# finmath/finmath-lib-cuda-extensions

Measured on AMD Instinct MI355X. Metric: Monte-Carlo path-ops/sec (fused RandomVariable stream), higher is better.
Workload: dtype f32

## Files before the change

### finmath-lib-cuda-extensions_amd/host/lmm.hpp

```cpp
#pragma once
#include <algorithm>
#include <chrono>
#include <cmath>
#include <cstdio>
#include <atomic>
#include <thread>
#include <cstdlib>
#include <functional>
#include <string>
#include <vector>

#include "random_variable.hpp"

namespace fmhost { namespace lmm {


inline const std::vector<double>& atmNormalVolatilities() {
    static const std::vector<double> v = {
        0.00151, 0.00169, 0.0021, 0.00248, 0.00291, 0.00329, 0.00365, 0.004, 0.00437, 0.00466, 0.00527, 0.00571,
        0.00604, 0.00625, 0.0016, 0.00174, 0.00217, 0.00264, 0.00314, 0.00355, 0.00398, 0.00433, 0.00469,
        0.00493, 0.00569, 0.00607, 0.00627, 0.00645, 0.00182, 0.00204, 0.00238, 0.00286, 0.00339, 0.00384,
        0.00424, 0.00456, 0.00488, 0.0052, 0.0059, 0.00623, 0.0064, 0.00654, 0.00205, 0.00235, 0.00272, 0.0032,
        0.00368, 0.00406, 0.00447, 0.00484, 0.00515, 0.00544, 0.00602, 0.00629, 0.0064, 0.00646, 0.00279,
        0.00319, 0.0036, 0.00396, 0.00436, 0.00469, 0.00503, 0.0053, 0.00557, 0.00582, 0.00616, 0.00628,
        0.00638, 0.00641, 0.00379, 0.00406, 0.00439, 0.00472, 0.00504, 0.00532, 0.0056, 0.00582, 0.00602,
        0.00617, 0.0063, 0.00636, 0.00638, 0.00639, 0.00471, 0.00489, 0.00511, 0.00539, 0.00563, 0.00583, 0.006,
        0.00618, 0.0063, 0.00644, 0.00641, 0.00638, 0.00635, 0.00634, 0.00544, 0.00557, 0.00572, 0.00591,
        0.00604, 0.00617, 0.0063, 0.00641, 0.00651, 0.00661, 0.00645, 0.00634, 0.00627, 0.00624, 0.00625,
        0.00632, 0.00638, 0.00644, 0.0065, 0.00655, 0.00661, 0.00667, 0.00672, 0.00673, 0.00634, 0.00614,
        0.00599, 0.00593, 0.00664, 0.00671, 0.00675, 0.00676, 0.00676, 0.00675, 0.00676, 0.00674, 0.00672,
        0.00669, 0.00616, 0.00586, 0.00569, 0.00558, 0.00647, 0.00651, 0.00651, 0.00651, 0.00652, 0.00649,
        0.00645, 0.0064, 0.00637, 0.00631, 0.00576, 0.00534, 0.00512, 0.00495, 0.00615, 0.0062, 0.00618,
        0.00613, 0.0061, 0.00607, 0.00602, 0.00596, 0.00591, 0.00586, 0.00536, 0.00491, 0.00469, 0.0045,
        0.00578, 0.00583, 0.00579, 0.00574, 0.00567, 0.00562, 0.00556, 0.00549, 0.00545, 0.00538, 0.00493,
        0.00453, 0.00435, 0.0042, 0.00542, 0.00547, 0.00539, 0.00532, 0.00522, 0.00516, 0.0051, 0.00504, 0.005,
        0.00495, 0.00454, 0.00418, 0.00404, 0.00394 };
    return v;
}
inline const std::vector<double>& atmExpiryYears() { static const std::vector<double> v = { 1.0 / 12, 0.25, 0.5, 1, 2, 3, 4, 5, 7, 10, 15, 20, 25, 30 }; return v; }
inline const std::vector<double>& atmTenorYears()  { static const std::vector<double> v = { 1, 2, 3, 4, 5, 6, 7, 8, 9, 10, 15, 20, 25, 30 }; return v; }

struct DiscountCurve {
    std::vector<double> t{ 0.0 }, logdf{ 0.0 };
    double df(double time) const {
        if (time <= 0.0) return 1.0;
        if (time >= t.back()) return std::exp(logdf.back());
        const size_t k = (size_t)(std::upper_bound(t.begin(), t.end(), time) - t.begin());
        const double w = (time - t[k - 1]) / (t[k] - t[k - 1]);
        return std::exp(logdf[k - 1] + w * (logdf[k] - logdf[k - 1]));
    }
    double forward(double fixing, double period) const { return (df(fixing) / df(fixing + period) - 1.0) / period; }
    static DiscountCurve bootstrap() {
        const double maturities[] = { 0.5, 1, 2, 3, 4, 5, 6, 7, 8, 9, 10, 11, 12, 15, 20, 25, 30, 35, 40, 45, 50 };
        const double rates[] = { -0.00216, -0.00208, -0.00222, -0.00216, -0.0019, -0.0014, -0.00072, 0.00011, 0.00103, 0.00196, 0.00285,
                                 0.00367, 0.0044, 0.00604, 0.00733, 0.00767, 0.00773, 0.00765, 0.00752, 0.007138, 0.007 };
        DiscountCurve c;
        for (int i = 0; i < 21; ++i) {
            const double M = maturities[i], r = rates[i];
            c.t.push_back(M); c.logdf.push_back(c.logdf.back());
            auto swapValue = [&](double ld) {
                c.logdf.back() = ld;
                double annuity = 0.0;
                if (M < 1.0) annuity = M * c.df(M);
                else for (double tp = 1.0; tp <= M + 1e-9; tp += 1.0) annuity += c.df(tp);
                return 1.0 - c.df(M) - r * annuity;
            };
            double lo = -3.0, hi = 1.0;
            for (int it = 0; it < 200; ++it) { const double mid = 0.5 * (lo + hi); if (swapValue(mid) > 0) lo = mid; else hi = mid; }
            c.logdf.back() = 0.5 * (lo + hi);
        }
        return c;
    }
};

struct Swaption {
    double exercise = 0; int numberOfPeriods = 0; double swapPeriodLength = 0.5;
    std::vector<double> swapTenor; double swaprate = 0, targetVolatility = 0, annuity = 0;
};

struct Market {
    DiscountCurve curve = DiscountCurve::bootstrap();
    double lastTime = 40.0, dt = 0.5;
    TimeDiscretization timeDiscretization{ 0.0, 80, 0.5 };
    std::vector<Swaption> swaptions;
    Market() {
        const auto& vols = atmNormalVolatilities();
        for (size_t e = 0; e < atmExpiryYears().size(); ++e)
            for (size_t k = 0; k < atmTenorYears().size(); ++k) {
                const double exercise = std::round(atmExpiryYears()[e] / 0.25) * 0.25, tenor = atmTenorYears()[k];
                if (exercise < 1.0) continue;
                if (exercise + tenor > lastTime + 1e-9) continue;
                Swaption s;
                s.exercise = exercise; s.numberOfPeriods = (int)std::lround(tenor / 0.5);
                for (int p = 0; p <= s.numberOfPeriods; ++p) s.swapTenor.push_back(exercise + p * 0.5);
                double floating = 0.0, annuity = 0.0;
                for (int p = 0; p < s.numberOfPeriods; ++p) {
                    const double d = curve.df(s.swapTenor[p + 1]);
                    floating += curve.forward(s.swapTenor[p], 0.5) * 0.5 * d; annuity += 0.5 * d;
                }
                s.swaprate = floating / annuity; s.annuity = annuity;
                s.targetVolatility = vols[e * atmTenorYears().size() + k];
                swaptions.push_back(std::move(s));
            }
    }
    int numberOfLibors() const { return timeDiscretization.getNumberOfTimeSteps(); }
};

struct VolatilityModel {
    std::vector<double> grid{ 0.0, 1.0, 2.0, 5.0, 10.0, 20.0, 30.0, 40.0 };
    std::vector<double> parameter = std::vector<double>(64, 0.50 / 100);
    int bin(double x) const { int k = 0; while (k < 7 && grid[(size_t)k] < x - 1e-12) ++k; return k; }
    int parameterIndex(double time, double maturity) const { return bin(time) * 8 + bin(maturity - time); }
    double volatility(double time, double maturity) const { return maturity <= time + 1e-12 ? 0.0 : parameter[(size_t)parameterIndex(time, maturity)]; }
    std::vector<int> activeParameters(const Market& m) const {
        std::vector<char> used(64, 0);
        const auto& td = m.timeDiscretization;
        for (int i = 0; i < td.getNumberOfTimeSteps(); ++i)
            for (int j = i + 1; j < m.numberOfLibors(); ++j) used[(size_t)parameterIndex(td.getTime(i), td.getTime(j))] = 1;
        std::vector<int> idx;
        for (int k = 0; k < 64; ++k) if (used[(size_t)k]) idx.push_back(k);
        return idx;
    }
};


struct Simulation {
    std::vector<std::vector<RV>> libor;
    std::vector<RV> numeraire;
};

struct Backend {
    const RandomVariableFactory* factory = nullptr;
    const BrownianMotion* brownianMotion = nullptr;
    std::function<void()> flush = [] {};
    std::function<void(bool)> hold = [](bool) {};
    std::function<long long()> launches = [] { return 0LL; };
    std::function<std::vector<double>(const std::vector<RV>&)> averages = [](const std::vector<RV>& v) {
        std::vector<double> a; for (const RV& x : v) a.push_back(x->getAverage()); return a; };
    std::function<std::function<std::vector<double>()>(const std::vector<RV>&)> averagesAsync;
    bool expectationsRunPending = false;
    std::function<void(const std::vector<RV>&)> valuesNotNeeded;
    int chunk = 7;
    int stepsPerLaunch = 4;
    std::function<std::vector<std::vector<RV>>(const std::vector<RV>& roots, const std::vector<RV>& leafFrom, const std::vector<std::vector<RV>>& leafTo,
                                               const std::vector<std::vector<double>>* scalars)> clone;
    std::function<std::vector<double>(const std::vector<RV>& roots)> recordedScalars;
    int jacobianBatch = 1;
    bool keepAllStates = false;
    int threads = 1;
};

inline std::vector<Simulation> simulateMany(const Market& m, const std::vector<const VolatilityModel*>& vols, const Backend& be, int lastTimeIndex,
                                            const std::vector<char>* keep = nullptr) {
    const auto& td = m.timeDiscretization;
    const int n = m.numberOfLibors();
    const double delta = m.dt;
    const size_t K = vols.size();
    std::vector<Simulation> sims(K);
    for (Simulation& sim : sims) {
        sim.libor.resize((size_t)lastTimeIndex + 1);
        sim.numeraire.resize((size_t)lastTimeIndex + 1);
        sim.libor[0].resize((size_t)n);
        for (int j = 0; j < n; ++j) sim.libor[0][(size_t)j] = be.factory->createRandomVariable(0.0, m.curve.forward(td.getTime(j), delta));
        sim.numeraire[0] = be.factory->createRandomVariable(0.0, 1.0);
    }
    std::vector<RV> factorSum(K);
    const int S = std::max(1, be.stepsPerLaunch);
    static int cloneChecks = 0;
    for (int i0 = 0; i0 < lastTimeIndex;) {
        int i1 = std::min(i0 + S, lastTimeIndex);
        static const bool endAtKept = std::getenv("FMHIP_LMM_GROUPS_END_AT_KEPT") && std::getenv("FMHIP_LMM_GROUPS_END_AT_KEPT")[0] == '1';
        if (keep && endAtKept) for (int s2 = i0 + 1; s2 < i1; ++s2) if ((*keep)[(size_t)s2]) { i1 = s2; break; }
        const bool cloning = K > 1 && S > 1 && keep && be.clone && i0 >= 2;
        const size_t Krec = cloning ? 1 : K;
        if (S > 1) be.hold(true);
        for (int i = i0; i < i1; ++i) {
            const double t = td.getTime(i), dt = td.getTimeStep(i);
            const RV dW = be.brownianMotion->getBrownianIncrement(i, 0);
            for (size_t k = 0; k < Krec; ++k) {
                auto& cur = sims[k].libor[(size_t)i];
                auto& nxt = sims[k].libor[(size_t)i + 1];
                nxt.resize((size_t)n);
                for (int j = 0; j <= i && j < n; ++j) nxt[(size_t)j] = cur[(size_t)j];
                factorSum[k] = nullptr;
            }
            for (int j0 = i + 1; j0 < n; j0 += be.chunk) {
                const int j1 = std::min(n, j0 + be.chunk);
                for (size_t k = 0; k < Krec; ++k) {
                    auto& cur = sims[k].libor[(size_t)i];
                    auto& nxt = sims[k].libor[(size_t)i + 1];
                    for (int j = j0; j < j1; ++j) {
                        const double lambda = vols[k]->volatility(t, td.getTime(j));
                        const RV& L = cur[(size_t)j];
                        const RV transform = be.factory->createRandomVariable(lambda * delta)->discount(L, delta);
                        factorSum[k] = factorSum[k] ? factorSum[k]->add(transform) : transform;
                        const RV drift = factorSum[k]->mult(lambda);
                        nxt[(size_t)j] = L->addProduct(drift, dt)->addProduct(dW, lambda);
                    }
                }
                if (S == 1 && j1 - j0 == be.chunk) be.flush();
            }
            for (size_t k = 0; k < Krec; ++k)
                sims[k].numeraire[(size_t)i + 1] = sims[k].numeraire[(size_t)i]->accrue(sims[k].libor[(size_t)i][(size_t)i], delta);
            for (size_t k = 0; k < Krec; ++k) factorSum[k] = nullptr;
        }
        if (cloning) {
            std::vector<RV> roots, leafFrom;
            for (int j = i0 + 1; j < n; ++j) roots.push_back(sims[0].libor[(size_t)i1][(size_t)j]);
            for (int i = i0; i < i1; ++i) roots.push_back(sims[0].numeraire[(size_t)i + 1]);
            for (int s2 = i0 + 1; s2 < i1; ++s2)
                if (!keep || (*keep)[(size_t)s2]) for (int j = s2; j < n; ++j) roots.push_back(sims[0].libor[(size_t)s2][(size_t)j]);
            for (int j = i0; j < n; ++j) leafFrom.push_back(sims[0].libor[(size_t)i0][(size_t)j]);
            leafFrom.push_back(sims[0].numeraire[(size_t)i0]);
            auto scalarsOf = [&](const VolatilityModel& vol) {
                std::vector<double> sc;
                for (int i = i0; i < i1; ++i) {
                    const double t = td.getTime(i), dt = td.getTimeStep(i);
                    for (int j = i + 1; j < n; ++j) {
                        const double lambda = vol.volatility(t, td.getTime(j));
                        sc.push_back(delta); sc.push_back(1.0); sc.push_back(lambda * delta); sc.push_back(lambda); sc.push_back(dt); sc.push_back(lambda);
                    }
                    sc.push_back(delta);
                }
                return sc;
            };
            if (cloneChecks < 64 && be.recordedScalars) {
                ++cloneChecks;
                if (be.recordedScalars(roots) != scalarsOf(*vols[0])) throw std::runtime_error("lmm: the scalar list of the replicated Euler steps does not match the recording");
            }
            std::vector<std::vector<RV>> leafTo(K - 1);
            std::vector<std::vector<double>> scalars(K - 1);
            for (size_t k = 1; k < K; ++k) {
                for (int j = i0; j < n; ++j) leafTo[k - 1].push_back(sims[k].libor[(size_t)i0][(size_t)j]);
                leafTo[k - 1].push_back(sims[k].numeraire[(size_t)i0]);
                scalars[k - 1] = scalarsOf(*vols[k]);
            }
            const std::vector<std::vector<RV>> copies = be.clone(roots, leafFrom, leafTo, &scalars);
            for (size_t k = 1; k < K; ++k) {
                auto& nxt = sims[k].libor[(size_t)i1];
                nxt.resize((size_t)n);
                for (int j = 0; j <= i0 && j < n; ++j) nxt[(size_t)j] = sims[k].libor[(size_t)i0][(size_t)j];
                size_t r = 0;
                for (int j = i0 + 1; j < n; ++j) nxt[(size_t)j] = copies[k - 1][r++];
                for (int i = i0; i < i1; ++i) sims[k].numeraire[(size_t)i + 1] = copies[k - 1][r++];
                for (int s2 = i0 + 1; s2 < i1; ++s2)
                    if (!keep || (*keep)[(size_t)s2]) { auto& mid = sims[k].libor[(size_t)s2]; mid.resize((size_t)n); for (int j = s2; j < n; ++j) mid[(size_t)j] = copies[k - 1][r++]; }
            }
        }
        if (keep)
            for (int i = i0; i < i1; ++i)
                if (!(*keep)[(size_t)i])
                    for (size_t k = 0; k < K; ++k) { sims[k].libor[(size_t)i].clear(); sims[k].libor[(size_t)i].shrink_to_fit(); }
        if (S > 1) be.hold(false);
        be.flush();
        i0 = i1;
    }
    return sims;
}

inline Simulation simulate(const Market& m, const VolatilityModel& vol, const Backend& be, int lastTimeIndex) {
    return std::move(simulateMany(m, { &vol }, be, lastTimeIndex)[0]);
}

inline RV swaptionValue(const Market& m, const Simulation& sim, const Swaption& s) {
    const auto& td = m.timeDiscretization;
    const int exerciseIndex = td.getTimeIndex(s.exercise);
    RV value;
    for (int p = s.numberOfPeriods - 1; p >= 0; --p) {
        const int j = td.getTimeIndex(s.swapTenor[(size_t)p]);
        const RV& libor = sim.libor[(size_t)exerciseIndex][(size_t)j];
        const RV payoff = libor->sub(s.swaprate)->mult(s.swapPeriodLength);
        value = (value ? value->add(payoff) : payoff)->discount(libor, s.swapPeriodLength);
    }
    return value->floor(0.0)->div(sim.numeraire[(size_t)exerciseIndex]);
}
inline double bachelierAtmImpliedVolatility(double optionValue, double optionMaturity, double annuity) {
    return optionValue * std::sqrt(2.0 * 3.14159265358979323846) / (annuity * std::sqrt(optionMaturity));
}

struct Valuation { std::vector<double> modelVolatility; double seconds_simulation = 0, seconds_valuation = 0; long long launches_simulation = 0, launches_valuation = 0; };

struct PendingValuations {
    std::vector<std::function<std::vector<double>()>> expectations;
    std::vector<Valuation> out;
};

inline std::vector<Valuation> evaluateManyFinish(const Market& m, PendingValuations& p) {
    for (size_t k = 0; k < p.out.size(); ++k) {
        const std::vector<double> optionValues = p.expectations[k]();
        for (size_t q = 0; q < m.swaptions.size(); ++q)
            p.out[k].modelVolatility.push_back(bachelierAtmImpliedVolatility(optionValues[q], m.swaptions[q].exercise, m.swaptions[q].annuity));
    }
    return std::move(p.out);
}

inline PendingValuations evaluateManyBegin(const Market& m, const std::vector<const VolatilityModel*>& vols, const Backend& be) {
    using clk = std::chrono::steady_clock;
    const size_t K = vols.size();
    PendingValuations pending;
    std::vector<Valuation>& out = pending.out;
    out.resize(K);
    int lastIndex = 0;
    for (const Swaption& s : m.swaptions) lastIndex = std::max(lastIndex, m.timeDiscretization.getTimeIndex(s.exercise));
    const auto t0 = clk::now();
    const long long l0 = be.launches();
    std::vector<char> keep((size_t)lastIndex + 1, 0);
    for (const Swaption& s : m.swaptions) keep[(size_t)m.timeDiscretization.getTimeIndex(s.exercise)] = 1;
    const std::vector<Simulation> sims = simulateMany(m, vols, be, lastIndex, be.keepAllStates ? nullptr : &keep);
    const auto t1 = clk::now();
    const long long l1 = be.launches();
    std::vector<std::vector<RV>> values(K);
    if (K > 1 && be.clone) {
        be.hold(true);
        values[0].reserve(m.swaptions.size());
        for (const Swaption& s : m.swaptions) values[0].push_back(swaptionValue(m, sims[0], s));
        std::vector<RV> leafFrom;
        std::vector<std::vector<RV>> leafTo(K - 1);
        for (int e = 0; e <= lastIndex; ++e) {
            if (!keep[(size_t)e]) continue;
            for (size_t k = 0; k < K; ++k) {
                std::vector<RV>& dst = k == 0 ? leafFrom : leafTo[k - 1];
                for (int j = e; j < m.numberOfLibors(); ++j) dst.push_back(sims[k].libor[(size_t)e][(size_t)j]);
                dst.push_back(sims[k].numeraire[(size_t)e]);
            }
        }
        const std::vector<std::vector<RV>> copies = be.clone(values[0], leafFrom, leafTo, nullptr);
        for (size_t k = 1; k < K; ++k) values[k] = copies[k - 1];
        be.hold(false);
        if (!(be.averagesAsync && be.expectationsRunPending)) be.flush();
    } else
    for (size_t k = 0; k < K; ++k) {
        be.hold(true);
        values[k].reserve(m.swaptions.size());
        for (const Swaption& s : m.swaptions) values[k].push_back(swaptionValue(m, sims[k], s));
        be.hold(false);
        if (!(be.averagesAsync && be.expectationsRunPending)) be.flush();
    }
    if (be.valuesNotNeeded) for (size_t k = 0; k < K; ++k) be.valuesNotNeeded(values[k]);
    for (size_t k = 0; k < K; ++k) {
        if (be.averagesAsync) pending.expectations.push_back(be.averagesAsync(values[k]));
        else { const std::vector<double> now = be.averages(values[k]); pending.expectations.push_back([now] { return now; }); }
    }
    const auto t2 = clk::now();
    for (size_t k = 0; k < K; ++k) {
        out[k].launches_simulation = (l1 - l0) / (long long)K; out[k].launches_valuation = (be.launches() - l1) / (long long)K;
        out[k].seconds_simulation = std::chrono::duration<double>(t1 - t0).count() / (double)K;
        out[k].seconds_valuation = std::chrono::duration<double>(t2 - t1).count() / (double)K;
    }
    return pending;
}

inline std::vector<Valuation> evaluateMany(const Market& m, const std::vector<const VolatilityModel*>& vols, const Backend& be) {
    PendingValuations p = evaluateManyBegin(m, vols, be);
    return evaluateManyFinish(m, p);
}

inline Valuation evaluate(const Market& m, const VolatilityModel& vol, const Backend& be) {
    return std::move(evaluateMany(m, { &vol }, be)[0]);
}


struct CalibrationResult {
    VolatilityModel model; int iterations = 0, evaluations = 0;
    double meanDeviation = 0, rmsDeviation = 0, initialRms = 0, seconds = 0, seconds_simulation = 0, seconds_valuation = 0;
    std::vector<double> modelVolatility;
};

inline bool solveSymmetric(std::vector<double> A, std::vector<double> b, int n, std::vector<double>& x) {
    for (int c = 0; c < n; ++c) {
        int piv = c;
        for (int r = c + 1; r < n; ++r) if (std::fabs(A[(size_t)r * n + c]) > std::fabs(A[(size_t)piv * n + c])) piv = r;
        if (std::fabs(A[(size_t)piv * n + c]) < 1e-300) return false;
        if (piv != c) { for (int k = 0; k < n; ++k) std::swap(A[(size_t)c * n + k], A[(size_t)piv * n + k]); std::swap(b[(size_t)c], b[(size_t)piv]); }
        for (int r = c + 1; r < n; ++r) {
            const double f = A[(size_t)r * n + c] / A[(size_t)c * n + c];
            for (int k = c; k < n; ++k) A[(size_t)r * n + k] -= f * A[(size_t)c * n + k];
            b[(size_t)r] -= f * b[(size_t)c];
        }
    }
    x.assign((size_t)n, 0.0);
    for (int r = n - 1; r >= 0; --r) { double s = b[(size_t)r]; for (int k = r + 1; k < n; ++k) s -= A[(size_t)r * n + k] * x[(size_t)k]; x[(size_t)r] = s / A[(size_t)r * n + r]; }
    return true;
}

inline CalibrationResult calibrate(const Market& m, const Backend& be, int maxIterations = 200, double accuracy = 1e-7,
                                   double lambda = 0.1, double parameterStep = 1e-4, bool verbose = false) {
    using clk = std::chrono::steady_clock;
    const auto start = clk::now();
    CalibrationResult res;
    VolatilityModel vol;
    const std::vector<int> active = vol.activeParameters(m);
    const int np = (int)active.size(), nr = (int)m.swaptions.size();
    auto residuals = [&](const VolatilityModel& v, std::vector<double>& r, std::vector<double>* modelVols) {
        const Valuation val = evaluate(m, v, be);
        res.evaluations++; res.seconds_simulation += val.seconds_simulation; res.seconds_valuation += val.seconds_valuation;
        r.resize((size_t)nr);
        for (int k = 0; k < nr; ++k) r[(size_t)k] = val.modelVolatility[(size_t)k] - m.swaptions[(size_t)k].targetVolatility;
        if (modelVols) *modelVols = val.modelVolatility;
    };
    auto sumsq = [](const std::vector<double>& r) { double s = 0; for (double x : r) s += x * x; return s; };
    std::vector<double> r, rTrial, modelVols;
    residuals(vol, r, &modelVols);
    double err = sumsq(r);
    res.initialRms = std::sqrt(err / nr);
    for (int it = 0; it < maxIterations; ++it) {
        std::vector<double> J((size_t)nr * np);
        struct InFlight { int a0 = 0, a1 = 0; std::vector<VolatilityModel> bumped; PendingValuations pending; bool valid = false; };
        auto collect = [&](InFlight& f) {
            if (!f.valid) return;
            const std::vector<Valuation> vals = evaluateManyFinish(m, f.pending);
            for (int a = f.a0; a < f.a1; ++a) {
                const Valuation& val = vals[(size_t)(a - f.a0)];
                res.evaluations++; res.seconds_simulation += val.seconds_simulation; res.seconds_valuation += val.seconds_valuation;
                for (int k = 0; k < nr; ++k) J[(size_t)k * np + a] = (val.modelVolatility[(size_t)k] - m.swaptions[(size_t)k].targetVolatility - r[(size_t)k]) / parameterStep;
            }
            f.valid = false;
        };
        if (be.threads > 1 && be.jacobianBatch <= 1) {
            const auto tj0 = clk::now();
            std::vector<Valuation> column((size_t)np);
            std::vector<std::string> failures((size_t)be.threads);
            std::atomic<int> next{ 0 };
            std::vector<std::thread> pool;
            for (int t = 0; t < be.threads; ++t)
                pool.emplace_back([&, t] {
                    try {
                        for (int a = next.fetch_add(1); a < np; a = next.fetch_add(1)) {
                            VolatilityModel bumped = vol;
                            bumped.parameter[(size_t)active[(size_t)a]] += parameterStep;
                            column[(size_t)a] = evaluate(m, bumped, be);
                        }
                    } catch (const std::exception& e) { failures[(size_t)t] = e.what(); }
                });
            for (std::thread& th : pool) th.join();
            if (std::getenv("FMHIP_LMM_TIMELINE")) std::fprintf(stderr, "[lmm timeline] iteration %d: %d columns on %d threads, %.3f … %.3f ms\n", it, np, be.threads, std::chrono::duration<double, std::milli>(tj0 - start).count(), std::chrono::duration<double, std::milli>(clk::now() - start).count());
            for (const std::string& f : failures) if (!f.empty()) throw std::runtime_error("a Jacobian column failed: " + f);
            for (int a = 0; a < np; ++a) {
                const Valuation& val = column[(size_t)a];
                res.evaluations++; res.seconds_simulation += val.seconds_simulation; res.seconds_valuation += val.seconds_valuation;
                for (int k = 0; k < nr; ++k) J[(size_t)k * np + a] = (val.modelVolatility[(size_t)k] - m.swaptions[(size_t)k].targetVolatility - r[(size_t)k]) / parameterStep;
            }
        } else {
        InFlight previous;
        for (int a0 = 0; a0 < np; a0 += std::max(1, be.jacobianBatch)) {
            const int a1 = std::min(np, a0 + std::max(1, be.jacobianBatch));
            InFlight current;
            current.a0 = a0; current.a1 = a1;
            current.bumped.assign((size_t)(a1 - a0), vol);
            std::vector<const VolatilityModel*> ptrs;
            for (int a = a0; a < a1; ++a) { current.bumped[(size_t)(a - a0)].parameter[(size_t)active[(size_t)a]] += parameterStep; ptrs.push_back(&current.bumped[(size_t)(a - a0)]); }
            static const bool timeline = std::getenv("FMHIP_LMM_TIMELINE") != nullptr;
            const auto tb0 = clk::now();
            try { current.pending = evaluateManyBegin(m, ptrs, be); current.valid = true; }
            catch (const std::exception& e) {
                if (ptrs.size() == 1 || std::string(e.what()).find("allocation") == std::string::npos) throw;
                if (verbose) std::fprintf(stderr, "  batch of %zu bumps does not fit (%s): evaluating them one at a time\n", ptrs.size(), e.what());
                be.flush();
                collect(previous);
                for (int a = a0; a < a1; ++a) {
                    const Valuation val = evaluate(m, current.bumped[(size_t)(a - a0)], be);
                    res.evaluations++; res.seconds_simulation += val.seconds_simulation; res.seconds_valuation += val.seconds_valuation;
                    for (int k = 0; k < nr; ++k) J[(size_t)k * np + a] = (val.modelVolatility[(size_t)k] - m.swaptions[(size_t)k].targetVolatility - r[(size_t)k]) / parameterStep;
                }
                continue;
            }
            const auto tb1 = clk::now();
            collect(previous);
            if (timeline) std::fprintf(stderr, "[lmm timeline] iteration %d batch from %d: begin %.3f … %.3f ms, previous collected at %.3f ms\n", it, a0,
                                       std::chrono::duration<double, std::milli>(tb0 - start).count(), std::chrono::duration<double, std::milli>(tb1 - start).count(),
                                       std::chrono::duration<double, std::milli>(clk::now() - start).count());
            previous = std::move(current);
        }
        collect(previous);
        }
        std::vector<double> JtJ((size_t)np * np, 0.0), Jtr((size_t)np, 0.0);
        for (int a = 0; a < np; ++a) {
            for (int b = 0; b < np; ++b) { double s = 0; for (int k = 0; k < nr; ++k) s += J[(size_t)k * np + a] * J[(size_t)k * np + b]; JtJ[(size_t)a * np + b] = s; }
            double s = 0; for (int k = 0; k < nr; ++k) s += J[(size_t)k * np + a] * r[(size_t)k]; Jtr[(size_t)a] = -s;
        }
        bool improved = false;
        for (int attempt = 0; attempt < 8 && !improved; ++attempt) {
            std::vector<double> A = JtJ, step;
            for (int a = 0; a < np; ++a) A[(size_t)a * np + a] += lambda * std::max(JtJ[(size_t)a * np + a], 1e-12);
            if (!solveSymmetric(A, Jtr, np, step)) { lambda *= 4; continue; }
            VolatilityModel v = vol;
            for (int a = 0; a < np; ++a) v.parameter[(size_t)active[(size_t)a]] += step[(size_t)a];
            std::vector<double> mv;
            const auto tt0 = clk::now();
            residuals(v, rTrial, &mv);
            static const bool timeline2 = std::getenv("FMHIP_LMM_TIMELINE") != nullptr;
            if (timeline2) std::fprintf(stderr, "[lmm timeline] iteration %d trial %d: %.3f … %.3f ms\n", it, attempt, std::chrono::duration<double, std::milli>(tt0 - start).count(),
                                        std::chrono::duration<double, std::milli>(clk::now() - start).count());
            const double e = sumsq(rTrial);
            if (e < err) { improved = true; const double rel = (err - e) / err; vol = v; r = rTrial; err = e; modelVols = mv; lambda = std::max(lambda / 3.0, 1e-9); if (rel < accuracy) it = maxIterations; }
            else lambda *= 4.0;
        }
        res.iterations++;
        if (verbose) std::fprintf(stderr, "  LM iteration %d: rms %.6e  lambda %.3g  evaluations %d\n", res.iterations, std::sqrt(err / nr), lambda, res.evaluations);
        if (!improved || std::sqrt(err / nr) < accuracy) break;
    }
    res.model = vol; res.modelVolatility = modelVols;
    double sum = 0; for (double x : r) sum += x;
    res.meanDeviation = sum / nr; res.rmsDeviation = std::sqrt(err / nr);
    res.seconds = std::chrono::duration<double>(clk::now() - start).count();
    return res;
}

}}
```

### finmath-lib-cuda-extensions_amd/host/lmm_hip_main.cpp

```cpp
#include <fstream>
#include <thread>
#include <csignal>
#include <execinfo.h>
#include <unistd.h>
#include <rccl/rccl.h>
#include "lmm_main_common.hpp"
#include "hip_backend.hpp"
using namespace fmhost;

static void ncclCheck(ncclResult_t r, const char* what) {
    if (r != ncclSuccess) throw std::runtime_error(std::string(what) + ": " + ncclGetErrorString(r));
}

static void fatalSignal(int sig) {
    void* frames[64];
    const int n = backtrace(frames, 64);
    const char msg[] = "lmm_hip: fatal signal, call stack:\n";
    (void)!write(2, msg, sizeof msg - 1);
    backtrace_symbols_fd(frames, n, 2);
    signal(sig, SIG_DFL);
    raise(sig);
}

int main(int argc, char** argv) {
    if (std::getenv("FMHIP_BACKTRACE")) { signal(SIGABRT, fatalSignal); signal(SIGSEGV, fatalSignal); signal(SIGBUS, fatalSignal); }
    const lmm::Options o = lmm::parseOptions(argc, argv);
    try {
        if (!o.devices.empty()) check(fmhip_init_devices(o.devices.data(), (int)o.devices.size()));
        else check(fmhip_init(-1));
        check(fmhip_set_fusion(1, nullptr));
        RandomVariableHipFactory factory;
        lmm::Market m;
        const int64_t pathOffset = o.pathOffset + (int64_t)o.rank * o.paths;
        BrownianMotionHip philox(m.timeDiscretization, 1, o.paths, o.seed, pathOffset);
        BrownianMotionFromMersenneRandomNumbers mersenne(m.timeDiscretization, 1, o.paths, (int)o.seed, &factory);
        if (o.brownian == "mersenne" && o.world > 1) throw std::runtime_error("--brownian mersenne is a sequential stream: not available with --world > 1 (mersenne-device is)");
        BrownianMotionFromMersenneRandomNumbersHip mersenneDevice(m.timeDiscretization, 1, o.paths, (int)o.seed, pathOffset);
        lmm::Backend be = makeHipBackend(&factory, (o.brownian == "mersenne") ? static_cast<const BrownianMotion*>(&mersenne)
                                                 : (o.brownian == "mersenne-device") ? static_cast<const BrownianMotion*>(&mersenneDevice) : &philox,
                                         o.chunk, o.stepsPerLaunch, o.jacobianBatch);

        if (o.finmathLike) {
            be.flush = [] {}; be.hold = [](bool) {}; be.clone = nullptr; be.recordedScalars = nullptr; be.averagesAsync = nullptr; be.expectationsRunPending = false;
            be.averages = [](const std::vector<RV>& v) { std::vector<double> a; for (const RV& x : v) a.push_back(x->getAverage()); return a; };
            be.jacobianBatch = 1; be.stepsPerLaunch = 1; be.chunk = 1 << 30; be.keepAllStates = true;
            if (o.threads > 1) {
                if (!o.devices.empty() || o.world > 1) throw std::runtime_error("--threads: one device, one process");
                check(fmhip_set_thread_engines(1, nullptr));
                be.threads = o.threads;
            }
        } else if (o.threads > 1) throw std::runtime_error("--threads belongs to --finmath-like (the native driver batches its Jacobian columns instead)");
        if (o.releaseLagMs > 0.0 || o.releaseLagBytes > 0) ReleaseLag::instance().start(o.releaseLagMs, (size_t)o.releaseLagBytes);
        ncclComm_t comm = nullptr;
        std::vector<std::pair<double*, hipEvent_t>> sparePinned;
        fmhip_vec sums = 0;
        long long collectives = 0;
        double collective_seconds = 0.0;
        if (o.world > 1 || !o.ncclIdFile.empty()) {
            if (o.ncclIdFile.empty()) throw std::runtime_error("--world needs --nccl-id-file");
            struct IdFile { uint64_t magic, nonce; ncclUniqueId id; } rec{};
            const uint64_t MAGIC = 0x464d4e43434c4944ull;
            if (o.rank == 0) {
                std::remove(o.ncclIdFile.c_str());
                rec.magic = MAGIC; rec.nonce = (uint64_t)o.ncclNonce;
                ncclCheck(ncclGetUniqueId(&rec.id), "ncclGetUniqueId");
                { std::ofstream f(o.ncclIdFile + ".tmp", std::ios::binary); f.write((const char*)&rec, sizeof rec); }
                std::rename((o.ncclIdFile + ".tmp").c_str(), o.ncclIdFile.c_str());
            } else {
                for (int tries = 0; ; ++tries) {
                    std::ifstream f(o.ncclIdFile, std::ios::binary);
                    if (f && f.read((char*)&rec, sizeof rec) && f.gcount() == (std::streamsize)sizeof rec && rec.magic == MAGIC && rec.nonce == (uint64_t)o.ncclNonce) break;
                    if (tries > 6000) throw std::runtime_error("timed out waiting for " + o.ncclIdFile);
                    std::this_thread::sleep_for(std::chrono::milliseconds(10));
                }
            }
            const ncclUniqueId id = rec.id;
            ncclCheck(ncclCommInitRank(&comm, o.world, id, o.rank), "ncclCommInitRank");
            if (o.rank == 0) std::remove(o.ncclIdFile.c_str());
            const int count = (int)m.swaptions.size();
            check(fmhip_vec_create_uninitialized((int64_t)count * 8 * o.world, &sums));
            void* stream = nullptr; check(fmhip_get_stream(&stream));
            const int64_t totalPaths = (int64_t)o.world * o.paths;
            const int world = o.world, rank = o.rank;
            struct Flight {
                fmhip_vec dev = 0; double* host = nullptr; hipEvent_t ev = nullptr;
                std::vector<std::pair<double*, hipEvent_t>>* spare = nullptr;
                ~Flight() { if (dev) fmhip_vec_release(dev); if (host && ev && spare) spare->push_back({ host, ev }); }
            };
            std::vector<std::pair<double*, hipEvent_t>>* const spare = &sparePinned;
            { const char* e = std::getenv("FMHIP_LMM_SHARDED_FROM_LAUNCHES"); be.expectationsRunPending = !(e && e[0] == '0'); }
            be.averagesAsync = [=, &collectives, &collective_seconds](const std::vector<RV>& v) -> std::function<std::vector<double>()> {
                std::vector<fmhip_vec> h;
                for (const RV& x : v) {
                    auto p = dynamic_cast<const RandomVariableHip*>(x.get());
                    if (!p || p->isDeterministic()) throw std::runtime_error("sharded expectation of a non-device value");
                    h.push_back(p->deviceVector().handle());
                }
                if ((int)h.size() != count) throw std::runtime_error("sharded expectation: unexpected product count");
                auto f = std::make_shared<Flight>();
                const size_t doubles = (size_t)count * 4 * (size_t)world;
                check(fmhip_vec_create_uninitialized((int64_t)doubles * 2, &f->dev));
                f->spare = spare;
                if (!spare->empty()) { f->host = spare->back().first; f->ev = spare->back().second; spare->pop_back(); }
                else if (hipHostMalloc((void**)&f->host, doubles * 8, hipHostMallocDefault) != hipSuccess || hipEventCreateWithFlags(&f->ev, hipEventDisableTiming) != hipSuccess)
                    throw std::runtime_error("pinned memory / event for a sharded expectation");
                void* dev = nullptr; check(fmhip_vec_device_ptr(f->dev, &dev));
                double* all = (double*)dev;
                check(fmhip_reduce_moments_batch_device(h.data(), count, nullptr, all + (size_t)rank * count * 4));
                ncclCheck(ncclAllGather(all + (size_t)rank * count * 4, all, (size_t)count * 4, ncclDouble, comm, (hipStream_t)stream), "ncclAllGather");
                if (hipMemcpyAsync(f->host, all, doubles * 8, hipMemcpyDeviceToHost, (hipStream_t)stream) != hipSuccess || hipEventRecord(f->ev, (hipStream_t)stream) != hipSuccess)
                    throw std::runtime_error("enqueueing the read-back of a sharded expectation");
                ++collectives;
                return [f, count, world, totalPaths, &collective_seconds] {
                    const auto t0 = std::chrono::steady_clock::now();
                    if (hipEventSynchronize(f->ev) != hipSuccess) throw std::runtime_error("waiting for a sharded expectation");
                    collective_seconds += std::chrono::duration<double>(std::chrono::steady_clock::now() - t0).count();
                    std::vector<double> out((size_t)count);
                    for (int k = 0; k < count; ++k) {
                        double total = 0.0;
                        for (int r = 0; r < world; ++r) total += f->host[((size_t)r * count + k) * 4];
                        out[(size_t)k] = total / (double)totalPaths;
                    }
                    return out;
                };
            };
            be.averages = [=, &collectives, &collective_seconds](const std::vector<RV>& v) {
                std::vector<fmhip_vec> h;
                for (const RV& x : v) {
                    auto p = dynamic_cast<const RandomVariableHip*>(x.get());
                    if (!p || p->isDeterministic()) throw std::runtime_error("sharded expectation of a non-device value");
                    h.push_back(p->deviceVector().handle());
                }
                if ((int)h.size() != count) throw std::runtime_error("sharded expectation: unexpected product count");
                void* dev = nullptr; check(fmhip_vec_device_ptr(sums, &dev));
                double* all = (double*)dev;
                check(fmhip_reduce_moments_batch_device(h.data(), count, nullptr, all + (size_t)rank * count * 4));
                const auto t0 = std::chrono::steady_clock::now();
                ncclCheck(ncclAllGather(all + (size_t)rank * count * 4, all, (size_t)count * 4, ncclDouble, comm, (hipStream_t)stream), "ncclAllGather");
                ++collectives;
                std::vector<float> raw((size_t)count * 8 * world);
                check(fmhip_vec_read_float(sums, raw.data(), (int64_t)raw.size()));
                collective_seconds += std::chrono::duration<double>(std::chrono::steady_clock::now() - t0).count();
                std::vector<double> out((size_t)count);
                for (int k = 0; k < count; ++k) {
                    double total = 0.0;
                    for (int r = 0; r < world; ++r) { double s; std::memcpy(&s, &raw[((size_t)r * count + k) * 8], 8); total += s; }
                    out[(size_t)k] = total / (double)totalPaths;
                }
                return out;
            };
        }

        if (o.mode == "evaluate" && o.warmupEvaluations > 0) {
            lmm::VolatilityModel vol;
            (void)lmm::evaluateMany(m, std::vector<const lmm::VolatilityModel*>((size_t)o.warmupEvaluations, &vol), be);
            check(fmhip_jit_wait());
        }
        fmhip_pool_stats_t s0; check(fmhip_pool_stats(&s0));
        int64_t bytes0 = 0; check(fmhip_traffic_stats(&bytes0, nullptr));
        if (o.profile) check(fmhip_profile_enable(1));
        auto extra = [&] {
            fmhip_pool_stats_t s; check(fmhip_pool_stats(&s));
            char name[128] = { 0 }; int cus = 0; int64_t hbm = 0; fmhip_device_info(name, 128, &cus, &hbm);
            int64_t jc = 0, jf = 0, jp = 0, jd = 0; double js = 0.0; fmhip_jit_stats(&jc, &jf, &jp, &js, &jd);
            int64_t bytes1 = 0, jl = 0; fmhip_traffic_stats(&bytes1, &jl);
            std::string prof;
            if (o.profile) {
                double ms = 0.0; int64_t nl = 0; fmhip_profile_read(&ms, &nl);
                char pb[256];
                std::snprintf(pb, sizeof pb, ", \"profiled_launches\": %lld, \"kernel_ms_total\": %.3f, \"achieved_GBps\": %.1f",
                              (long long)nl, ms, ms > 0 ? (double)(bytes1 - bytes0) / (ms * 1e-3) / 1e9 : 0.0);
                prof = pb;
            }
            char buf[768];
            std::snprintf(buf, sizeof buf, ", \"kernel_launches\": %lld, \"path_ops\": %.6e, \"device_bytes_reserved\": %lld, \"device\": \"%s\", "
                          "\"world\": %d, \"rank\": %d, \"total_paths\": %lld, \"rccl_collectives\": %lld, \"rccl_collective_seconds\": %.6f, "
                          "\"specialised_kernels\": %lld, \"specialisations_from_disk_cache\": %lld, \"specialisations_pending\": %lld, \"specialisation_seconds\": %.3f, "
                          "\"algorithmic_bytes\": %lld, \"specialised_launches\": %lld",
                          (long long)(s.n_kernel_launches - s0.n_kernel_launches), (double)(s.n_ops_executed - s0.n_ops_executed) * (double)o.paths,
                          (long long)s.bytes_reserved, name, o.world, o.rank, (long long)o.world * (long long)o.paths, collectives, collective_seconds,
                          (long long)jc, (long long)jd, (long long)jp, js, (long long)(bytes1 - bytes0), (long long)jl);
            std::string lag;
            if (ReleaseLag::instance().on()) {
                const ReleaseLag::Stats ls = ReleaseLag::instance().stats();
                char lb[384];
                std::snprintf(lb, sizeof lb, ", \"release_lag\": {\"collect_every_ms\": %.3f, \"collect_at_bytes\": %lld, \"handles_queued\": %lld, \"handles_released\": %lld, "
                              "\"collections\": %lld, \"collections_forced_by_out_of_memory\": %lld, \"peak_dead_handles\": %lld}",
                              o.releaseLagMs, o.releaseLagBytes, ls.queued, ls.released, ls.collections, ls.forcedCollections, ls.peakQueue);
                lag = lb;
            }
            fmhip_engine_stats_t es; check(fmhip_engine_stats(&es));
            char eb[768];
            std::snprintf(eb, sizeof eb, ", \"engine\": {\"interpreter_launches\": %lld, \"algorithmic_bytes_written\": %lld, \"values_deferred\": %lld, \"values_deferred_now\": %lld, "
                          "\"values_demanded\": %lld, \"peak_bytes_reserved\": %lld, \"late_releases_while_waiting\": %lld, \"late_releases_at_once\": %lld, \"late_release_seconds\": %.3f, "
                          "\"merged_launches\": %lld, \"merged_chains\": %lld, \"common_rows\": %lld, \"rolled_launches\": %lld}",
                          (long long)es.interpreter_launches, (long long)es.algorithmic_bytes_written, (long long)es.values_deferred, (long long)es.values_deferred_now,
                          (long long)es.values_demanded, (long long)es.peak_bytes_reserved, (long long)es.late_releases_while_waiting, (long long)es.late_releases_at_once, (double)es.late_release_nanoseconds * 1e-9,
                          (long long)es.merged_launches, (long long)es.merged_chains, (long long)es.common_rows, (long long)es.rolled_launches);
            return std::string(buf) + prof + lag + eb;
        };
        if (o.rank == 0) lmm::runAndReport(o, be, "hip", extra);
        else { lmm::Options quiet = o; quiet.verbose = false; lmm::runAndReport(quiet, be, "hip", extra); }
        if (sums) fmhip_vec_release(sums);
        ReleaseLag::instance().stop();
        be = lmm::Backend();
        for (auto& pe : sparePinned) { (void)hipHostFree(pe.first); (void)hipEventDestroy(pe.second); }
        if (comm) ncclCommDestroy(comm);
        check(fmhip_shutdown());
    } catch (const std::exception& e) { std::fprintf(stderr, "lmm_hip[rank %d]: %s\n", o.rank, e.what()); return 1; }
    return 0;
}
```

### finmath-lib-cuda-extensions_amd/host/lmm_main_common.hpp

```cpp
#pragma once
#include <vector>
#include <cstdlib>
#include <cstring>
#include <string>
#include "lmm.hpp"

namespace fmhost { namespace lmm {

struct Options {
    int64_t paths = 10000; int64_t seed = 31415; int maxIterations = 200; std::string mode = "calibrate"; bool verbose = false;
    int64_t pathOffset = 0; int evaluations = 1;
    int warmupEvaluations = 0;
    int world = 1, rank = 0; std::string ncclIdFile; long long ncclNonce = 0;
    std::vector<int> devices;
    int chunk = 0;
    int stepsPerLaunch = 0;
    int jacobianBatch = 0;
    std::string brownian = "philox";
    int threads = 1;
    double releaseLagMs = 0.0;
    long long releaseLagBytes = 0;
    bool finmathLike = false;
    bool profile = false;
};
inline Options parseOptions(int argc, char** argv) {
    Options o;
    for (int i = 1; i < argc; ++i) {
        const std::string a = argv[i];
        auto next = [&]() -> const char* { if (i + 1 >= argc) { std::fprintf(stderr, "missing value for %s\n", a.c_str()); std::exit(2); } return argv[++i]; };
        if (a == "--paths") o.paths = std::atoll(next());
        else if (a == "--seed") o.seed = std::atoll(next());
        else if (a == "--max-iterations") o.maxIterations = std::atoi(next());
        else if (a == "--mode") o.mode = next();
        else if (a == "--evaluations") o.evaluations = std::atoi(next());
        else if (a == "--warmup-evaluations") o.warmupEvaluations = std::atoi(next());
        else if (a == "--path-offset") o.pathOffset = std::atoll(next());
        else if (a == "--world") o.world = std::atoi(next());
        else if (a == "--devices") { std::string list = next(); size_t p0 = 0; while (p0 <= list.size()) { const size_t q = list.find(',', p0); o.devices.push_back(std::atoi(list.substr(p0, q == std::string::npos ? std::string::npos : q - p0).c_str())); if (q == std::string::npos) break; p0 = q + 1; } }
        else if (a == "--rank") o.rank = std::atoi(next());
        else if (a == "--nccl-id-file") o.ncclIdFile = next();
        else if (a == "--nccl-nonce") o.ncclNonce = std::atoll(next());
        else if (a == "--profile") o.profile = true;
        else if (a == "--finmath-like") o.finmathLike = true;
        else if (a == "--threads") o.threads = std::atoi(next());
        else if (a == "--release-lag") o.releaseLagMs = std::atof(next());
        else if (a == "--release-lag-bytes") o.releaseLagBytes = std::atoll(next());
        else if (a == "--brownian") o.brownian = next();
        else if (a == "--jacobian-batch") o.jacobianBatch = std::atoi(next());
        else if (a == "--chunk") o.chunk = std::atoi(next());
        else if (a == "--steps-per-launch") o.stepsPerLaunch = std::atoi(next());
        else if (a == "--verbose") o.verbose = true;
        else { std::fprintf(stderr, "unknown option %s\n", a.c_str()); std::exit(2); }
    }
    return o;
}

inline void runAndReport(const Options& o, const Backend& be, const char* backendName, const std::function<std::string()>& extraJson) {
    Market m;
    if (o.mode == "evaluate") {
        VolatilityModel vol;
        Valuation v;
        double sim = 0, val = 0;
        const int K = std::max(1, o.jacobianBatch);
        for (int k = 0; k < o.evaluations; k += K) {
            const int kk = std::min(K, o.evaluations - k);
            const std::vector<Valuation> vs = evaluateMany(m, std::vector<const VolatilityModel*>((size_t)kk, &vol), be);
            for (const Valuation& x : vs) { sim += x.seconds_simulation; val += x.seconds_valuation; }
            v = vs.back();
        }
        std::printf("{\"backend\": \"%s\", \"mode\": \"evaluate\", \"paths\": %lld, \"swaptions\": %zu, \"evaluations\": %d, "
                    "\"seconds_simulation_per_evaluation\": %.6f, \"seconds_valuation_per_evaluation\": %.6f, \"launches_simulation\": %lld, \"launches_valuation\": %lld%s, \"model_volatility\": [",
                    backendName, (long long)o.paths, m.swaptions.size(), o.evaluations, sim / o.evaluations, val / o.evaluations, v.launches_simulation, v.launches_valuation, extraJson().c_str());
        for (size_t k = 0; k < v.modelVolatility.size(); ++k) std::printf("%s%.17g", k ? ", " : "", v.modelVolatility[k]);
        std::printf("]}\n");
        return;
    }
    const CalibrationResult r = calibrate(m, be, o.maxIterations, 1e-7, 0.1, 1e-4, o.verbose);
    std::printf("{\"backend\": \"%s\", \"mode\": \"calibrate\", \"paths\": %lld, \"swaptions\": %zu, \"active_parameters\": %zu, "
                "\"iterations\": %d, \"evaluations\": %d, \"seconds\": %.4f, \"seconds_simulation\": %.4f, \"seconds_valuation\": %.4f, "
                "\"initial_rms\": %.6e, \"rms_deviation\": %.6e, \"mean_deviation\": %.6e%s, \"parameters\": [",
                backendName, (long long)o.paths, m.swaptions.size(), VolatilityModel().activeParameters(m).size(), r.iterations, r.evaluations,
                r.seconds, r.seconds_simulation, r.seconds_valuation, r.initialRms, r.rmsDeviation, r.meanDeviation, extraJson().c_str());
    for (size_t k = 0; k < r.model.parameter.size(); ++k) std::printf("%s%.17g", k ? ", " : "", r.model.parameter[k]);
    std::printf("]}\n");
}

}}
```

Before: 4220 billion.

## Restart Jacobian column simulations from base point at the first divergent Euler step

During calibration, each perturbed volatility model is compared against the base model to find the first time step where volatilities differ. Euler groups before that step reuse the base point's retained LIBOR and numeraire states. Columns that never diverge reuse the base option values, and only the swaptions affected are revalued. This is meant to skip redundant path simulation and valuation work in finite-difference Jacobians, at the cost of retaining group-start states in memory and handling variable product counts in the sharded reductions.

```diff
diff --git a/finmath-lib-cuda-extensions_amd/host/lmm.hpp b/finmath-lib-cuda-extensions_amd/host/lmm.hpp
--- a/finmath-lib-cuda-extensions_amd/host/lmm.hpp
+++ b/finmath-lib-cuda-extensions_amd/host/lmm.hpp
@@ -6,7 +6,10 @@
 #include <atomic>
 #include <thread>
 #include <cstdlib>
+#include <cstring>
 #include <functional>
+#include <limits>
+#include <memory>
 #include <string>
 #include <vector>
 
@@ -147,19 +150,74 @@
     std::function<std::vector<double>(const std::vector<RV>& roots)> recordedScalars;
     int jacobianBatch = 1;
     bool keepAllStates = false;
+    bool restartFromBase = true;
+    bool everySetReduces = false;
     int threads = 1;
 };
 
+
+constexpr int NEVER = std::numeric_limits<int>::max();
+
+inline int divergenceStep(const Market& m, const VolatilityModel& a, const VolatilityModel& b, int lastTimeIndex) {
+    const auto& td = m.timeDiscretization;
+    for (int d = 0; d < lastTimeIndex; ++d)
+        for (int j = d + 1; j < m.numberOfLibors(); ++j) {
+            const double x = a.volatility(td.getTime(d), td.getTime(j)), y = b.volatility(td.getTime(d), td.getTime(j));
+            if (std::memcmp(&x, &y, sizeof x) != 0) return d;
+        }
+    return NEVER;
+}
+
+inline bool groupsEndAtKept() {
+    static const bool on = std::getenv("FMHIP_LMM_GROUPS_END_AT_KEPT") && std::getenv("FMHIP_LMM_GROUPS_END_AT_KEPT")[0] == '1';
+    return on;
+}
+inline std::vector<int> eulerGroupStarts(const Backend& be, int lastTimeIndex, const std::vector<char>* keep) {
+    const int S = std::max(1, be.stepsPerLaunch);
+    std::vector<int> starts;
+    for (int i0 = 0; i0 < lastTimeIndex;) {
+        int i1 = std::min(i0 + S, lastTimeIndex);
+        if (keep && groupsEndAtKept()) for (int s2 = i0 + 1; s2 < i1; ++s2) if ((*keep)[(size_t)s2]) { i1 = s2; break; }
+        starts.push_back(i0);
+        i0 = i1;
+    }
+    starts.push_back(lastTimeIndex);
+    return starts;
+}
+
+struct BasePoint {
+    VolatilityModel model;
+    int lastTimeIndex = -1;
+    std::vector<int> groupStarts;
+    Simulation states;
+    std::vector<double> optionValues;
+    bool valid() const { return lastTimeIndex >= 0 && !optionValues.empty(); }
+};
+
 inline std::vector<Simulation> simulateMany(const Market& m, const std::vector<const VolatilityModel*>& vols, const Backend& be, int lastTimeIndex,
-                                            const std::vector<char>* keep = nullptr) {
+                                            const std::vector<char>* keep = nullptr, const BasePoint* base = nullptr, const std::vector<int>* diverges = nullptr,
+                                            bool retainGroupStarts = false, long long* groupsFromBase = nullptr) {
     const auto& td = m.timeDiscretization;
     const int n = m.numberOfLibors();
     const double delta = m.dt;
     const size_t K = vols.size();
+    const std::vector<int> starts = eulerGroupStarts(be, lastTimeIndex, keep);
+    std::vector<int> joinAt(K, 0);
+    if (base && diverges && base->lastTimeIndex == lastTimeIndex && base->groupStarts == starts)
+        for (size_t k = 0; k < K; ++k) {
+            const int d = (*diverges)[k];
+            if (d == NEVER) { joinAt[k] = NEVER; continue; }
+            size_t g = 0;
+            while (g + 2 < starts.size() && starts[g + 1] <= d) ++g;
+            joinAt[k] = starts[g];
+            if (groupsFromBase) *groupsFromBase += (long long)g;
+        }
     std::vector<Simulation> sims(K);
-    for (Simulation& sim : sims) {
+    for (size_t k = 0; k < K; ++k) {
+        Simulation& sim = sims[k];
         sim.libor.resize((size_t)lastTimeIndex + 1);
         sim.numeraire.resize((size_t)lastTimeIndex + 1);
+        if (joinAt[k] != 0) continue;
         sim.libor[0].resize((size_t)n);
         for (int j = 0; j < n; ++j) sim.libor[0][(size_t)j] = be.factory->createRandomVariable(0.0, m.curve.forward(td.getTime(j), delta));
         sim.numeraire[0] = be.factory->createRandomVariable(0.0, 1.0);
@@ -167,17 +225,25 @@
     std::vector<RV> factorSum(K);
     const int S = std::max(1, be.stepsPerLaunch);
     static int cloneChecks = 0;
-    for (int i0 = 0; i0 < lastTimeIndex;) {
-        int i1 = std::min(i0 + S, lastTimeIndex);
-        static const bool endAtKept = std::getenv("FMHIP_LMM_GROUPS_END_AT_KEPT") && std::getenv("FMHIP_LMM_GROUPS_END_AT_KEPT")[0] == '1';
-        if (keep && endAtKept) for (int s2 = i0 + 1; s2 < i1; ++s2) if ((*keep)[(size_t)s2]) { i1 = s2; break; }
-        const bool cloning = K > 1 && S > 1 && keep && be.clone && i0 >= 2;
-        const size_t Krec = cloning ? 1 : K;
+    for (size_t g = 0; g + 1 < starts.size(); ++g) {
+        const int i0 = starts[g], i1 = starts[g + 1];
+        std::vector<size_t> active;
+        for (size_t k = 0; k < K; ++k) {
+            if (joinAt[k] == i0 && i0 > 0) {
+                if (base->states.libor[(size_t)i0].size() != (size_t)n || !base->states.numeraire[(size_t)i0]) throw std::runtime_error("lmm: the base point has no state at a group start");
+                sims[k].libor[(size_t)i0] = base->states.libor[(size_t)i0];
+                sims[k].numeraire[(size_t)i0] = base->states.numeraire[(size_t)i0];
+            }
+            if (joinAt[k] <= i0) active.push_back(k);
+        }
+        if (active.empty()) continue;
+        const bool cloning = active.size() > 1 && S > 1 && keep && be.clone && i0 >= 2;
+        const std::vector<size_t> recorded = cloning ? std::vector<size_t>{ active[0] } : active;
         if (S > 1) be.hold(true);
         for (int i = i0; i < i1; ++i) {
             const double t = td.getTime(i), dt = td.getTimeStep(i);
             const RV dW = be.brownianMotion->getBrownianIncrement(i, 0);
-            for (size_t k = 0; k < Krec; ++k) {
+            for (size_t k : recorded) {
                 auto& cur = sims[k].libor[(size_t)i];
                 auto& nxt = sims[k].libor[(size_t)i + 1];
                 nxt.resize((size_t)n);
@@ -186,7 +252,7 @@
             }
             for (int j0 = i + 1; j0 < n; j0 += be.chunk) {
                 const int j1 = std::min(n, j0 + be.chunk);
-                for (size_t k = 0; k < Krec; ++k) {
+                for (size_t k : recorded) {
                     auto& cur = sims[k].libor[(size_t)i];
                     auto& nxt = sims[k].libor[(size_t)i + 1];
                     for (int j = j0; j < j1; ++j) {
@@ -200,18 +266,19 @@
                 }
                 if (S == 1 && j1 - j0 == be.chunk) be.flush();
             }
-            for (size_t k = 0; k < Krec; ++k)
+            for (size_t k : recorded)
                 sims[k].numeraire[(size_t)i + 1] = sims[k].numeraire[(size_t)i]->accrue(sims[k].libor[(size_t)i][(size_t)i], delta);
-            for (size_t k = 0; k < Krec; ++k) factorSum[k] = nullptr;
+            for (size_t k : recorded) factorSum[k] = nullptr;
         }
         if (cloning) {
+            const Simulation& first = sims[active[0]];
             std::vector<RV> roots, leafFrom;
-            for (int j = i0 + 1; j < n; ++j) roots.push_back(sims[0].libor[(size_t)i1][(size_t)j]);
-            for (int i = i0; i < i1; ++i) roots.push_back(sims[0].numeraire[(size_t)i + 1]);
+            for (int j = i0 + 1; j < n; ++j) roots.push_back(first.libor[(size_t)i1][(size_t)j]);
+            for (int i = i0; i < i1; ++i) roots.push_back(first.numeraire[(size_t)i + 1]);
             for (int s2 = i0 + 1; s2 < i1; ++s2)
-                if (!keep || (*keep)[(size_t)s2]) for (int j = s2; j < n; ++j) roots.push_back(sims[0].libor[(size_t)s2][(size_t)j]);
-            for (int j = i0; j < n; ++j) leafFrom.push_back(sims[0].libor[(size_t)i0][(size_t)j]);
-            leafFrom.push_back(sims[0].numeraire[(size_t)i0]);
+                if (!keep || (*keep)[(size_t)s2]) for (int j = s2; j < n; ++j) roots.push_back(first.libor[(size_t)s2][(size_t)j]);
+            for (int j = i0; j < n; ++j) leafFrom.push_back(first.libor[(size_t)i0][(size_t)j]);
+            leafFrom.push_back(first.numeraire[(size_t)i0]);
             auto scalarsOf = [&](const VolatilityModel& vol) {
                 std::vector<double> sc;
                 for (int i = i0; i < i1; ++i) {
@@ -226,34 +293,36 @@
             };
             if (cloneChecks < 64 && be.recordedScalars) {
                 ++cloneChecks;
-                if (be.recordedScalars(roots) != scalarsOf(*vols[0])) throw std::runtime_error("lmm: the scalar list of the replicated Euler steps does not match the recording");
-            }
-            std::vector<std::vector<RV>> leafTo(K - 1);
-            std::vector<std::vector<double>> scalars(K - 1);
-            for (size_t k = 1; k < K; ++k) {
-                for (int j = i0; j < n; ++j) leafTo[k - 1].push_back(sims[k].libor[(size_t)i0][(size_t)j]);
-                leafTo[k - 1].push_back(sims[k].numeraire[(size_t)i0]);
-                scalars[k - 1] = scalarsOf(*vols[k]);
+                if (be.recordedScalars(roots) != scalarsOf(*vols[active[0]])) throw std::runtime_error("lmm: the scalar list of the replicated Euler steps does not match the recording");
+            }
+            const size_t C = active.size() - 1;
+            std::vector<std::vector<RV>> leafTo(C);
+            std::vector<std::vector<double>> scalars(C);
+            for (size_t c = 0; c < C; ++c) {
+                const size_t k = active[c + 1];
+                for (int j = i0; j < n; ++j) leafTo[c].push_back(sims[k].libor[(size_t)i0][(size_t)j]);
+                leafTo[c].push_back(sims[k].numeraire[(size_t)i0]);
+                scalars[c] = scalarsOf(*vols[k]);
             }
             const std::vector<std::vector<RV>> copies = be.clone(roots, leafFrom, leafTo, &scalars);
-            for (size_t k = 1; k < K; ++k) {
+            for (size_t c = 0; c < C; ++c) {
+                const size_t k = active[c + 1];
                 auto& nxt = sims[k].libor[(size_t)i1];
                 nxt.resize((size_t)n);
                 for (int j = 0; j <= i0 && j < n; ++j) nxt[(size_t)j] = sims[k].libor[(size_t)i0][(size_t)j];
                 size_t r = 0;
-                for (int j = i0 + 1; j < n; ++j) nxt[(size_t)j] = copies[k - 1][r++];
-                for (int i = i0; i < i1; ++i) sims[k].numeraire[(size_t)i + 1] = copies[k - 1][r++];
+                for (int j = i0 + 1; j < n; ++j) nxt[(size_t)j] = copies[c][r++];
+                for (int i = i0; i < i1; ++i) sims[k].numeraire[(size_t)i + 1] = copies[c][r++];
                 for (int s2 = i0 + 1; s2 < i1; ++s2)
-                    if (!keep || (*keep)[(size_t)s2]) { auto& mid = sims[k].libor[(size_t)s2]; mid.resize((size_t)n); for (int j = s2; j < n; ++j) mid[(size_t)j] = copies[k - 1][r++]; }
+                    if (!keep || (*keep)[(size_t)s2]) { auto& mid = sims[k].libor[(size_t)s2]; mid.resize((size_t)n); for (int j = s2; j < n; ++j) mid[(size_t)j] = copies[c][r++]; }
             }
         }
         if (keep)
             for (int i = i0; i < i1; ++i)
-                if (!(*keep)[(size_t)i])
+                if (!(*keep)[(size_t)i] && !(retainGroupStarts && i == i0))
                     for (size_t k = 0; k < K; ++k) { sims[k].libor[(size_t)i].clear(); sims[k].libor[(size_t)i].shrink_to_fit(); }
         if (S > 1) be.hold(false);
         be.flush();
-        i0 = i1;
     }
     return sims;
 }
@@ -278,68 +347,140 @@
     return optionValue * std::sqrt(2.0 * 3.14159265358979323846) / (annuity * std::sqrt(optionMaturity));
 }
 
-struct Valuation { std::vector<double> modelVolatility; double seconds_simulation = 0, seconds_valuation = 0; long long launches_simulation = 0, launches_valuation = 0; };
+struct Valuation { std::vector<double> modelVolatility, optionValues; double seconds_simulation = 0, seconds_valuation = 0; long long launches_simulation = 0, launches_valuation = 0; };
 
 struct PendingValuations {
     std::vector<std::function<std::vector<double>()>> expectations;
     std::vector<Valuation> out;
+    long long eulerGroupsFromBase = 0, expectationsFromBase = 0;
 };
 
 inline std::vector<Valuation> evaluateManyFinish(const Market& m, PendingValuations& p) {
     for (size_t k = 0; k < p.out.size(); ++k) {
-        const std::vector<double> optionValues = p.expectations[k]();
+        p.out[k].optionValues = p.expectations[k]();
         for (size_t q = 0; q < m.swaptions.size(); ++q)
-            p.out[k].modelVolatility.push_back(bachelierAtmImpliedVolatility(optionValues[q], m.swaptions[q].exercise, m.swaptions[q].annuity));
+            p.out[k].modelVolatility.push_back(bachelierAtmImpliedVolatility(p.out[k].optionValues[q], m.swaptions[q].exercise, m.swaptions[q].annuity));
     }
     return std::move(p.out);
 }
 
-inline PendingValuations evaluateManyBegin(const Market& m, const std::vector<const VolatilityModel*>& vols, const Backend& be) {
+inline int lastExerciseIndex(const Market& m) {
+    int lastIndex = 0;
+    for (const Swaption& s : m.swaptions) lastIndex = std::max(lastIndex, m.timeDiscretization.getTimeIndex(s.exercise));
+    return lastIndex;
+}
+
+inline PendingValuations evaluateManyBegin(const Market& m, const std::vector<const VolatilityModel*>& vols, const Backend& be,
+                                           const BasePoint* base = nullptr, BasePoint* retain = nullptr) {
     using clk = std::chrono::steady_clock;
-    const size_t K = vols.size();
+    const size_t K = vols.size(), Q = m.swaptions.size();
     PendingValuations pending;
     std::vector<Valuation>& out = pending.out;
     out.resize(K);
-    int lastIndex = 0;
-    for (const Swaption& s : m.swaptions) lastIndex = std::max(lastIndex, m.timeDiscretization.getTimeIndex(s.exercise));
+    const int lastIndex = lastExerciseIndex(m);
     const auto t0 = clk::now();
     const long long l0 = be.launches();
     std::vector<char> keep((size_t)lastIndex + 1, 0);
-    for (const Swaption& s : m.swaptions) keep[(size_t)m.timeDiscretization.getTimeIndex(s.exercise)] = 1;
-    const std::vector<Simulation> sims = simulateMany(m, vols, be, lastIndex, be.keepAllStates ? nullptr : &keep);
+    std::vector<int> exerciseIndex(Q);
+    for (size_t q = 0; q < Q; ++q) { exerciseIndex[q] = m.timeDiscretization.getTimeIndex(m.swaptions[q].exercise); keep[(size_t)exerciseIndex[q]] = 1; }
+    const std::vector<char>* keepList = be.keepAllStates ? nullptr : &keep;
+    if (!keepList) retain = nullptr;
+    if (base && !(keepList && base->valid() && base->lastTimeIndex == lastIndex && base->optionValues.size() == Q
+                  && base->groupStarts == eulerGroupStarts(be, lastIndex, keepList))) base = nullptr;
+    std::vector<size_t> live;
+    std::vector<int> diverges;
+    std::vector<const VolatilityModel*> liveVols;
+    for (size_t k = 0; k < K; ++k) {
+        int d = base ? divergenceStep(m, base->model, *vols[k], lastIndex) : -1;
+        if (d == NEVER && be.everySetReduces) d = lastIndex - 1;
+        if (d == NEVER) { pending.expectationsFromBase += (long long)Q; continue; }
+        live.push_back(k); diverges.push_back(d); liveVols.push_back(vols[k]);
+    }
+    const size_t KL = live.size();
+    const std::vector<Simulation> sims = KL == 0 ? std::vector<Simulation>()
+        : simulateMany(m, liveVols, be, lastIndex, keepList, base, base ? &diverges : nullptr, retain != nullptr, &pending.eulerGroupsFromBase);
     const auto t1 = clk::now();
     const long long l1 = be.launches();
-    std::vector<std::vector<RV>> values(K);
-    if (K > 1 && be.clone) {
+    auto valued = [&](size_t c, size_t q) { return diverges[c] < exerciseIndex[q]; };
+    std::vector<std::vector<RV>> values(KL, std::vector<RV>(Q));
+    if (KL > 1 && be.clone) {
         be.hold(true);
-        values[0].reserve(m.swaptions.size());
-        for (const Swaption& s : m.swaptions) values[0].push_back(swaptionValue(m, sims[0], s));
-        std::vector<RV> leafFrom;
-        std::vector<std::vector<RV>> leafTo(K - 1);
-        for (int e = 0; e <= lastIndex; ++e) {
-            if (!keep[(size_t)e]) continue;
-            for (size_t k = 0; k < K; ++k) {
-                std::vector<RV>& dst = k == 0 ? leafFrom : leafTo[k - 1];
-                for (int j = e; j < m.numberOfLibors(); ++j) dst.push_back(sims[k].libor[(size_t)e][(size_t)j]);
-                dst.push_back(sims[k].numeraire[(size_t)e]);
-            }
-        }
-        const std::vector<std::vector<RV>> copies = be.clone(values[0], leafFrom, leafTo, nullptr);
-        for (size_t k = 1; k < K; ++k) values[k] = copies[k - 1];
+        std::vector<int> dates;
+        for (int e = 0; e <= lastIndex; ++e) if (keep[(size_t)e]) dates.push_back(e);
+        auto setsAt = [&](int e) { std::vector<size_t> a; for (size_t c = 0; c < KL; ++c) if (diverges[c] < e) a.push_back(c); return a; };
+        for (size_t d0 = 0; d0 < dates.size();) {
+            const std::vector<size_t> sets = setsAt(dates[d0]);
+            size_t d1 = d0 + 1;
+            while (d1 < dates.size() && setsAt(dates[d1]) == sets) ++d1;
+            const int eFrom = dates[d0], eTo = dates[d1 - 1];
+            d0 = d1;
+            if (sets.empty()) continue;
+            std::vector<RV> roots;
+            std::vector<size_t> rootProduct;
+            for (size_t q = 0; q < Q; ++q)
+                if (exerciseIndex[q] >= eFrom && exerciseIndex[q] <= eTo) { values[sets[0]][q] = swaptionValue(m, sims[sets[0]], m.swaptions[q]); roots.push_back(values[sets[0]][q]); rootProduct.push_back(q); }
+            if (sets.size() == 1) continue;
+            std::vector<RV> leafFrom;
+            std::vector<std::vector<RV>> leafTo(sets.size() - 1);
+            for (int e = eFrom; e <= eTo; ++e) {
+                if (!keep[(size_t)e]) continue;
+                for (size_t i = 0; i < sets.size(); ++i) {
+                    std::vector<RV>& dst = i == 0 ? leafFrom : leafTo[i - 1];
+                    for (int j = e; j < m.numberOfLibors(); ++j) dst.push_back(sims[sets[i]].libor[(size_t)e][(size_t)j]);
+                    dst.push_back(sims[sets[i]].numeraire[(size_t)e]);
+                }
+            }
+            const std::vector<std::vector<RV>> copies = be.clone(roots, leafFrom, leafTo, nullptr);
+            for (size_t i = 1; i < sets.size(); ++i)
+                for (size_t r = 0; r < roots.size(); ++r) values[sets[i]][rootProduct[r]] = copies[i - 1][r];
+        }
         be.hold(false);
         if (!(be.averagesAsync && be.expectationsRunPending)) be.flush();
     } else
-    for (size_t k = 0; k < K; ++k) {
+    for (size_t c = 0; c < KL; ++c) {
         be.hold(true);
-        values[k].reserve(m.swaptions.size());
-        for (const Swaption& s : m.swaptions) values[k].push_back(swaptionValue(m, sims[k], s));
+        for (size_t q = 0; q < Q; ++q) if (valued(c, q)) values[c][q] = swaptionValue(m, sims[c], m.swaptions[q]);
         be.hold(false);
         if (!(be.averagesAsync && be.expectationsRunPending)) be.flush();
     }
-    if (be.valuesNotNeeded) for (size_t k = 0; k < K; ++k) be.valuesNotNeeded(values[k]);
-    for (size_t k = 0; k < K; ++k) {
-        if (be.averagesAsync) pending.expectations.push_back(be.averagesAsync(values[k]));
-        else { const std::vector<double> now = be.averages(values[k]); pending.expectations.push_back([now] { return now; }); }
+    std::vector<std::vector<RV>> own(KL);
+    std::vector<std::vector<size_t>> ownProduct(KL);
+    for (size_t c = 0; c < KL; ++c)
+        for (size_t q = 0; q < Q; ++q)
+            if (values[c][q]) { own[c].push_back(values[c][q]); ownProduct[c].push_back(q); }
+    values.clear();
+    if (be.valuesNotNeeded) for (size_t c = 0; c < KL; ++c) if (!own[c].empty()) be.valuesNotNeeded(own[c]);
+    const std::shared_ptr<const std::vector<double>> baseValues = base ? std::make_shared<const std::vector<double>>(base->optionValues) : nullptr;
+    pending.expectations.resize(K);
+    for (size_t k = 0; k < K; ++k) pending.expectations[k] = [baseValues] { return *baseValues; };
+    for (size_t c = 0; c < KL; ++c) {
+        pending.expectationsFromBase += (long long)(Q - own[c].size());
+        std::function<std::vector<double>()> part;
+        if (own[c].empty()) part = [] { return std::vector<double>(); };
+        else if (be.averagesAsync) part = be.averagesAsync(own[c]);
+        else { const std::vector<double> now = be.averages(own[c]); part = [now] { return now; }; }
+        const std::vector<size_t> where = ownProduct[c];
+        pending.expectations[live[c]] = [part, where, baseValues, Q] {
+            std::vector<double> all = baseValues ? *baseValues : std::vector<double>(Q, 0.0);
+            const std::vector<double> got = part();
+            for (size_t i = 0; i < where.size(); ++i) all[where[i]] = got[i];
+            return all;
+        };
+    }
+    if (retain && KL == 1 && K == 1) {
+        retain->model = *vols[0]; retain->lastTimeIndex = lastIndex; retain->groupStarts = eulerGroupStarts(be, lastIndex, keepList);
+        retain->optionValues.clear();
+        retain->states = Simulation();
+        retain->states.libor.resize((size_t)lastIndex + 1);
+        retain->states.numeraire.resize((size_t)lastIndex + 1);
+        std::vector<char> wanted = keep;
+        for (int i0 : retain->groupStarts) wanted[(size_t)i0] = 1;
+        for (int i = 0; i <= lastIndex; ++i) {
+            if (!wanted[(size_t)i]) continue;
+            retain->states.libor[(size_t)i] = sims[0].libor[(size_t)i];
+            for (int j = 0; j < i && j < (int)retain->states.libor[(size_t)i].size(); ++j) retain->states.libor[(size_t)i][(size_t)j] = nullptr;
+            retain->states.numeraire[(size_t)i] = sims[0].numeraire[(size_t)i];
+        }
     }
     const auto t2 = clk::now();
     for (size_t k = 0; k < K; ++k) {
@@ -364,6 +505,7 @@
     VolatilityModel model; int iterations = 0, evaluations = 0;
     double meanDeviation = 0, rmsDeviation = 0, initialRms = 0, seconds = 0, seconds_simulation = 0, seconds_valuation = 0;
     std::vector<double> modelVolatility;
+    long long jacobianColumnsNotSimulated = 0, eulerGroupsFromBase = 0, expectationsFromBase = 0;
 };
 
 inline bool solveSymmetric(std::vector<double> A, std::vector<double> b, int n, std::vector<double>& x) {
@@ -391,8 +533,14 @@
     VolatilityModel vol;
     const std::vector<int> active = vol.activeParameters(m);
     const int np = (int)active.size(), nr = (int)m.swaptions.size();
-    auto residuals = [&](const VolatilityModel& v, std::vector<double>& r, std::vector<double>* modelVols) {
-        const Valuation val = evaluate(m, v, be);
+    static const bool restartKnob = !(std::getenv("FMHIP_LMM_RESTART") && std::getenv("FMHIP_LMM_RESTART")[0] == '0');
+    const bool restart = restartKnob && be.restartFromBase && !be.keepAllStates && be.threads <= 1;
+    const int lastIndex = lastExerciseIndex(m);
+    BasePoint base, candidate;
+    auto residuals = [&](const VolatilityModel& v, std::vector<double>& r, std::vector<double>* modelVols, BasePoint* retain) {
+        PendingValuations p = evaluateManyBegin(m, { &v }, be, nullptr, retain);
+        const Valuation val = std::move(evaluateManyFinish(m, p)[0]);
+        if (retain) retain->optionValues = val.optionValues;
         res.evaluations++; res.seconds_simulation += val.seconds_simulation; res.seconds_valuation += val.seconds_valuation;
         r.resize((size_t)nr);
         for (int k = 0; k < nr; ++k) r[(size_t)k] = val.modelVolatility[(size_t)k] - m.swaptions[(size_t)k].targetVolatility;
@@ -400,17 +548,19 @@
     };
     auto sumsq = [](const std::vector<double>& r) { double s = 0; for (double x : r) s += x * x; return s; };
     std::vector<double> r, rTrial, modelVols;
-    residuals(vol, r, &modelVols);
+    residuals(vol, r, &modelVols, restart ? &base : nullptr);
     double err = sumsq(r);
     res.initialRms = std::sqrt(err / nr);
     for (int it = 0; it < maxIterations; ++it) {
         std::vector<double> J((size_t)nr * np);
-        struct InFlight { int a0 = 0, a1 = 0; std::vector<VolatilityModel> bumped; PendingValuations pending; bool valid = false; };
+        struct InFlight { std::vector<int> columns; std::vector<VolatilityModel> bumped; PendingValuations pending; bool valid = false; };
         auto collect = [&](InFlight& f) {
             if (!f.valid) return;
+            res.eulerGroupsFromBase += f.pending.eulerGroupsFromBase; res.expectationsFromBase += f.pending.expectationsFromBase;
             const std::vector<Valuation> vals = evaluateManyFinish(m, f.pending);
-            for (int a = f.a0; a < f.a1; ++a) {
-                const Valuation& val = vals[(size_t)(a - f.a0)];
+            for (size_t c = 0; c < f.columns.size(); ++c) {
+                const int a = f.columns[c];
+                const Valuation& val = vals[c];
                 res.evaluations++; res.seconds_simulation += val.seconds_simulation; res.seconds_valuation += val.seconds_valuation;
                 for (int k = 0; k < nr; ++k) J[(size_t)k * np + a] = (val.modelVolatility[(size_t)k] - m.swaptions[(size_t)k].targetVolatility - r[(size_t)k]) / parameterStep;
             }
@@ -441,24 +591,44 @@
                 for (int k = 0; k < nr; ++k) J[(size_t)k * np + a] = (val.modelVolatility[(size_t)k] - m.swaptions[(size_t)k].targetVolatility - r[(size_t)k]) / parameterStep;
             }
         } else {
+        const BasePoint* from = restart && base.valid() ? &base : nullptr;
+        std::vector<int> columns;
+        for (int a = 0; a < np; ++a) {
+            if (from) {
+                VolatilityModel bumped = vol;
+                bumped.parameter[(size_t)active[(size_t)a]] += parameterStep;
+                if (!be.everySetReduces && divergenceStep(m, from->model, bumped, lastIndex) == NEVER) {
+                    res.evaluations++; res.jacobianColumnsNotSimulated++; res.expectationsFromBase += nr;
+                    for (int k = 0; k < nr; ++k) {
+                        const double modelVolatility = bachelierAtmImpliedVolatility(from->optionValues[(size_t)k], m.swaptions[(size_t)k].exercise, m.swaptions[(size_t)k].annuity);
+                        J[(size_t)k * np + a] = (modelVolatility - m.swaptions[(size_t)k].targetVolatility - r[(size_t)k]) / parameterStep;
+                    }
+                    continue;
+                }
+            }
+            columns.push_back(a);
+        }
         InFlight previous;
-        for (int a0 = 0; a0 < np; a0 += std::max(1, be.jacobianBatch)) {
-            const int a1 = std::min(np, a0 + std::max(1, be.jacobianBatch));
+        const size_t batch = (size_t)std::max(1, be.jacobianBatch);
+        for (size_t c0 = 0; c0 < columns.size(); c0 += batch) {
+            const size_t c1 = std::min(columns.size(), c0 + batch);
+            const int a0 = columns[c0];
             InFlight current;
-            current.a0 = a0; current.a1 = a1;
-            current.bumped.assign((size_t)(a1 - a0), vol);
+            current.columns.assign(columns.begin() + (std::ptrdiff_t)c0, columns.begin() + (std::ptrdiff_t)c1);
+            current.bumped.assign(c1 - c0, vol);
             std::vector<const VolatilityModel*> ptrs;
-            for (int a = a0; a < a1; ++a) { current.bumped[(size_t)(a - a0)].parameter[(size_t)active[(size_t)a]] += parameterStep; ptrs.push_back(&current.bumped[(size_t)(a - a0)]); }
+            for (size_t c = c0; c < c1; ++c) { current.bumped[c - c0].parameter[(size_t)active[(size_t)columns[c]]] += parameterStep; ptrs.push_back(&current.bumped[c - c0]); }
             static const bool timeline = std::getenv("FMHIP_LMM_TIMELINE") != nullptr;
             const auto tb0 = clk::now();
-            try { current.pending = evaluateManyBegin(m, ptrs, be); current.valid = true; }
+            try { current.pending = evaluateManyBegin(m, ptrs, be, from); current.valid = true; }
             catch (const std::exception& e) {
                 if (ptrs.size() == 1 || std::string(e.what()).find("allocation") == std::string::npos) throw;
                 if (verbose) std::fprintf(stderr, "  batch of %zu bumps does not fit (%s): evaluating them one at a time\n", ptrs.size(), e.what());
                 be.flush();
                 collect(previous);
-                for (int a = a0; a < a1; ++a) {
-                    const Valuation val = evaluate(m, current.bumped[(size_t)(a - a0)], be);
+                for (size_t c = c0; c < c1; ++c) {
+                    const int a = columns[c];
+                    const Valuation val = evaluate(m, current.bumped[c - c0], be);
                     res.evaluations++; res.seconds_simulation += val.seconds_simulation; res.seconds_valuation += val.seconds_valuation;
                     for (int k = 0; k < nr; ++k) J[(size_t)k * np + a] = (val.modelVolatility[(size_t)k] - m.swaptions[(size_t)k].targetVolatility - r[(size_t)k]) / parameterStep;
                 }
@@ -487,11 +657,13 @@
             for (int a = 0; a < np; ++a) v.parameter[(size_t)active[(size_t)a]] += step[(size_t)a];
             std::vector<double> mv;
             const auto tt0 = clk::now();
-            residuals(v, rTrial, &mv);
+            residuals(v, rTrial, &mv, restart ? &candidate : nullptr);
             static const bool timeline2 = std::getenv("FMHIP_LMM_TIMELINE") != nullptr;
             if (timeline2) std::fprintf(stderr, "[lmm timeline] iteration %d trial %d: %.3f … %.3f ms\n", it, attempt, std::chrono::duration<double, std::milli>(tt0 - start).count(),
                                         std::chrono::duration<double, std::milli>(clk::now() - start).count());
             const double e = sumsq(rTrial);
+            if (e < err) base = std::move(candidate);
+            candidate = BasePoint();
             if (e < err) { improved = true; const double rel = (err - e) / err; vol = v; r = rTrial; err = e; modelVols = mv; lambda = std::max(lambda / 3.0, 1e-9); if (rel < accuracy) it = maxIterations; }
             else lambda *= 4.0;
         }
diff --git a/finmath-lib-cuda-extensions_amd/host/lmm_hip_main.cpp b/finmath-lib-cuda-extensions_amd/host/lmm_hip_main.cpp
--- a/finmath-lib-cuda-extensions_amd/host/lmm_hip_main.cpp
+++ b/finmath-lib-cuda-extensions_amd/host/lmm_hip_main.cpp
@@ -43,7 +43,7 @@
         if (o.finmathLike) {
             be.flush = [] {}; be.hold = [](bool) {}; be.clone = nullptr; be.recordedScalars = nullptr; be.averagesAsync = nullptr; be.expectationsRunPending = false;
             be.averages = [](const std::vector<RV>& v) { std::vector<double> a; for (const RV& x : v) a.push_back(x->getAverage()); return a; };
-            be.jacobianBatch = 1; be.stepsPerLaunch = 1; be.chunk = 1 << 30; be.keepAllStates = true;
+            be.jacobianBatch = 1; be.stepsPerLaunch = 1; be.chunk = 1 << 30; be.keepAllStates = true; be.restartFromBase = false;
             if (o.threads > 1) {
                 if (!o.devices.empty() || o.world > 1) throw std::runtime_error("--threads: one device, one process");
                 check(fmhip_set_thread_engines(1, nullptr));
@@ -89,6 +89,7 @@
             };
             std::vector<std::pair<double*, hipEvent_t>>* const spare = &sparePinned;
             { const char* e = std::getenv("FMHIP_LMM_SHARDED_FROM_LAUNCHES"); be.expectationsRunPending = !(e && e[0] == '0'); }
+            be.everySetReduces = true;
             be.averagesAsync = [=, &collectives, &collective_seconds](const std::vector<RV>& v) -> std::function<std::vector<double>()> {
                 std::vector<fmhip_vec> h;
                 for (const RV& x : v) {
@@ -96,7 +97,9 @@
                     if (!p || p->isDeterministic()) throw std::runtime_error("sharded expectation of a non-device value");
                     h.push_back(p->deviceVector().handle());
                 }
-                if ((int)h.size() != count) throw std::runtime_error("sharded expectation: unexpected product count");
+                const int cnt = (int)h.size();
+                if (cnt > count) throw std::runtime_error("sharded expectation: more products than the market has");
+                if (cnt == 0) return [] { return std::vector<double>(); };
                 auto f = std::make_shared<Flight>();
                 const size_t doubles = (size_t)count * 4 * (size_t)world;
                 check(fmhip_vec_create_uninitialized((int64_t)doubles * 2, &f->dev));
@@ -106,19 +109,19 @@
                     throw std::runtime_error("pinned memory / event for a sharded expectation");
                 void* dev = nullptr; check(fmhip_vec_device_ptr(f->dev, &dev));
                 double* all = (double*)dev;
-                check(fmhip_reduce_moments_batch_device(h.data(), count, nullptr, all + (size_t)rank * count * 4));
-                ncclCheck(ncclAllGather(all + (size_t)rank * count * 4, all, (size_t)count * 4, ncclDouble, comm, (hipStream_t)stream), "ncclAllGather");
-                if (hipMemcpyAsync(f->host, all, doubles * 8, hipMemcpyDeviceToHost, (hipStream_t)stream) != hipSuccess || hipEventRecord(f->ev, (hipStream_t)stream) != hipSuccess)
+                check(fmhip_reduce_moments_batch_device(h.data(), cnt, nullptr, all + (size_t)rank * cnt * 4));
+                ncclCheck(ncclAllGather(all + (size_t)rank * cnt * 4, all, (size_t)cnt * 4, ncclDouble, comm, (hipStream_t)stream), "ncclAllGather");
+                if (hipMemcpyAsync(f->host, all, (size_t)cnt * 4 * (size_t)world * 8, hipMemcpyDeviceToHost, (hipStream_t)stream) != hipSuccess || hipEventRecord(f->ev, (hipStream_t)stream) != hipSuccess)
                     throw std::runtime_error("enqueueing the read-back of a sharded expectation");
                 ++collectives;
-                return [f, count, world, totalPaths, &collective_seconds] {
+                return [f, cnt, world, totalPaths, &collective_seconds] {
                     const auto t0 = std::chrono::steady_clock::now();
                     if (hipEventSynchronize(f->ev) != hipSuccess) throw std::runtime_error("waiting for a sharded expectation");
                     collective_seconds += std::chrono::duration<double>(std::chrono::steady_clock::now() - t0).count();
-                    std::vector<double> out((size_t)count);
-                    for (int k = 0; k < count; ++k) {
+                    std::vector<double> out((size_t)cnt);
+                    for (int k = 0; k < cnt; ++k) {
                         double total = 0.0;
-                        for (int r = 0; r < world; ++r) total += f->host[((size_t)r * count + k) * 4];
+                        for (int r = 0; r < world; ++r) total += f->host[((size_t)r * cnt + k) * 4];
                         out[(size_t)k] = total / (double)totalPaths;
                     }
                     return out;
@@ -131,20 +134,22 @@
                     if (!p || p->isDeterministic()) throw std::runtime_error("sharded expectation of a non-device value");
                     h.push_back(p->deviceVector().handle());
                 }
-                if ((int)h.size() != count) throw std::runtime_error("sharded expectation: unexpected product count");
+                const int cnt = (int)h.size();
+                if (cnt > count) throw std::runtime_error("sharded expectation: more products than the market has");
+                if (cnt == 0) return std::vector<double>();
                 void* dev = nullptr; check(fmhip_vec_device_ptr(sums, &dev));
                 double* all = (double*)dev;
-                check(fmhip_reduce_moments_batch_device(h.data(), count, nullptr, all + (size_t)rank * count * 4));
+                check(fmhip_reduce_moments_batch_device(h.data(), cnt, nullptr, all + (size_t)rank * cnt * 4));
                 const auto t0 = std::chrono::steady_clock::now();
-                ncclCheck(ncclAllGather(all + (size_t)rank * count * 4, all, (size_t)count * 4, ncclDouble, comm, (hipStream_t)stream), "ncclAllGather");
+                ncclCheck(ncclAllGather(all + (size_t)rank * cnt * 4, all, (size_t)cnt * 4, ncclDouble, comm, (hipStream_t)stream), "ncclAllGather");
                 ++collectives;
                 std::vector<float> raw((size_t)count * 8 * world);
                 check(fmhip_vec_read_float(sums, raw.data(), (int64_t)raw.size()));
                 collective_seconds += std::chrono::duration<double>(std::chrono::steady_clock::now() - t0).count();
-                std::vector<double> out((size_t)count);
-                for (int k = 0; k < count; ++k) {
+                std::vector<double> out((size_t)cnt);
+                for (int k = 0; k < cnt; ++k) {
                     double total = 0.0;
-                    for (int r = 0; r < world; ++r) { double s; std::memcpy(&s, &raw[((size_t)r * count + k) * 8], 8); total += s; }
+                    for (int r = 0; r < world; ++r) { double s; std::memcpy(&s, &raw[((size_t)r * cnt + k) * 8], 8); total += s; }
                     out[(size_t)k] = total / (double)totalPaths;
                 }
                 return out;
diff --git a/finmath-lib-cuda-extensions_amd/host/lmm_main_common.hpp b/finmath-lib-cuda-extensions_amd/host/lmm_main_common.hpp
--- a/finmath-lib-cuda-extensions_amd/host/lmm_main_common.hpp
+++ b/finmath-lib-cuda-extensions_amd/host/lmm_main_common.hpp
@@ -78,9 +78,11 @@
     const CalibrationResult r = calibrate(m, be, o.maxIterations, 1e-7, 0.1, 1e-4, o.verbose);
     std::printf("{\"backend\": \"%s\", \"mode\": \"calibrate\", \"paths\": %lld, \"swaptions\": %zu, \"active_parameters\": %zu, "
                 "\"iterations\": %d, \"evaluations\": %d, \"seconds\": %.4f, \"seconds_simulation\": %.4f, \"seconds_valuation\": %.4f, "
-                "\"initial_rms\": %.6e, \"rms_deviation\": %.6e, \"mean_deviation\": %.6e%s, \"parameters\": [",
+                "\"initial_rms\": %.6e, \"rms_deviation\": %.6e, \"mean_deviation\": %.6e, "
+                "\"jacobian_columns_not_simulated\": %lld, \"euler_groups_from_base\": %lld, \"expectations_from_base\": %lld%s, \"parameters\": [",
                 backendName, (long long)o.paths, m.swaptions.size(), VolatilityModel().activeParameters(m).size(), r.iterations, r.evaluations,
-                r.seconds, r.seconds_simulation, r.seconds_valuation, r.initialRms, r.rmsDeviation, r.meanDeviation, extraJson().c_str());
+                r.seconds, r.seconds_simulation, r.seconds_valuation, r.initialRms, r.rmsDeviation, r.meanDeviation,
+                r.jacobianColumnsNotSimulated, r.eulerGroupsFromBase, r.expectationsFromBase, extraJson().c_str());
     for (size_t k = 0; k < r.model.parameter.size(); ++k) std::printf("%s%.17g", k ? ", " : "", r.model.parameter[k]);
     std::printf("]}\n");
 }
```

Measured after the change: 4273 billion (median of 3 runs). About the same (+1.3%).
